# eduardburlacu/DiTSep

Hardware: AMD Instinct MI355X
Metric: separated utterances/sec @ N=30, 2-spk 4 s mixtures (higher is better)
Workload: dtype fp16 (fp16 MFMA operands, fp32 accumulate)

## Files before the change

ditsep_amd/csrc/common.h:

```cpp
#pragma once
#include <hip/hip_runtime.h>
#include <stdint.h>

typedef unsigned short op16_t;
typedef __attribute__((ext_vector_type(8))) unsigned short op16x8;
typedef __attribute__((ext_vector_type(4))) unsigned short op16x4;
typedef __attribute__((ext_vector_type(8))) __bf16 bf16x8;
typedef __attribute__((ext_vector_type(8))) _Float16 f16x8;
typedef __attribute__((ext_vector_type(4))) float f32x4;

#define DSN_WAVE 64

#define DSN_PL(planes, f16) ((planes) | ((f16) << 4))
#define PL_COUNT(pl) ((pl)&3)
#define PL_F16(pl) ((pl) >> 4)

enum { DSN_ACT_NONE = 0, DSN_ACT_ELU = 1, DSN_ACT_SNAKE = 2, DSN_ACT_SILU = 3 };
enum { DSN_F32_NONE = 0, DSN_F32_TANH = 1 };

__device__ __forceinline__ float dsn_elu(float v) { return v > 0.f ? v : expm1f(v); }
__device__ __forceinline__ float dsn_silu(float v) { return v / (1.f + __expf(-v)); }
__device__ __forceinline__ float dsn_snake(float v, float alpha, float inv_beta) {
  float s = __sinf(v * alpha);
  return v + inv_beta * s * s;
}

#define DSN_F16_MAX 65504.f
__device__ __forceinline__ float dsn_sat16(float v) {
  const float c = __builtin_amdgcn_fmed3f(v, -DSN_F16_MAX, DSN_F16_MAX);
  return v != v ? v : c;
}
__device__ __forceinline__ op16_t to_op16(float v, int f16) {
  return f16 ? __builtin_bit_cast(unsigned short, (_Float16)dsn_sat16(v)) : __builtin_bit_cast(unsigned short, (__bf16)v);
}
__device__ __forceinline__ float from_op16(op16_t u, int f16) {
  return f16 ? (float)__builtin_bit_cast(_Float16, u) : (float)__builtin_bit_cast(__bf16, u);
// ... 131 lines not shown
```

ditsep_amd/csrc/engine.hip:

```cpp
#include <math.h>
#include <stdarg.h>
#include <stdio.h>
#include <stdlib.h>
#include <string.h>

#include <algorithm>
#include <map>
#include <numeric>
#include <set>
#include <stdexcept>
#include <string>
#include <vector>

#include "../../include/ditsep_hip.h"
#include "igemm.h"
#include "kernels.h"

namespace {

struct Err : std::runtime_error {
  int code;
  Err(int c, const std::string& m) : std::runtime_error(m), code(c) {}
};

// ... 1664 lines not shown
    if (ctx->fin_err_host && *ctx->fin_err_host) {
      *ctx->fin_err_host = 0;
      fail(DSN_EHIP, "a GroupNorm hand-off wait of an earlier call gave up (the workgroups of one conv were not resident "
                     "together): that call's results are invalid; DSN_NO_GN_FIN=1 selects the separate GroupNorm pass");
    }
    f();
    return DSN_OK;
  } catch (const Err& e) {
    ctx->err = e.what();
    return e.code;
  } catch (const std::exception& e) {
    ctx->err = e.what();
    return DSN_EINVAL;
  }
}
}

extern "C" {

dsn_ctx* dsn_create(const dsn_config* cfg) {
  try {
    if (!cfg) fail(DSN_EINVAL, "null config");
    if (cfg->precision < DSN_PREC_BF16 || cfg->precision > DSN_PREC_FP8)
      fail(DSN_EINVAL, "precision must be one of DSN_PREC_{BF16,BF16X3,FP16,FP16X3,FP8}");
    if (cfg->vae_n_blocks < 0 || cfg->vae_n_blocks > DSN_MAX_VAE_BLOCKS) fail(DSN_EINVAL, "bad vae_n_blocks");
    if (cfg->n_src < 1 || cfg->latent_dim % 32 != 0) fail(DSN_EINVAL, "bad n_src / latent_dim");
    if (cfg->score_kind == DSN_SCORE_DIT &&
        (cfg->dit_heads <= 0 || cfg->dit_embed_dim <= 0 || cfg->dit_embed_dim % cfg->dit_heads != 0 ||
         cfg->dit_embed_dim / cfg->dit_heads != 64))
      fail(DSN_EINVAL, "DiT: only 64-wide attention heads are implemented (embed_dim %d / %d heads = %d)",
           cfg->dit_embed_dim, cfg->dit_heads, cfg->dit_heads > 0 ? cfg->dit_embed_dim / cfg->dit_heads : 0);
// ... 1448 lines not shown
        d.X = t->x;
        d.b7 = t->bias;
        d.b1 = t->bias2;
        d.out_f32 = t->out_f32;
        d.out_planes = oplanes;
        d.out_ps = t->out_ps;
        d.act_mid = t->act;
        d.mid_a = t->act_a;
        d.mid_b = t->act_b;
        d.act_out = t->act_out;
        d.out_a = t->out_act_a;
        d.out_b = t->out_act_b;
        d.S = t->B;
        d.L = t->L;
        d.dil = t->dil;
        const hipError_t e = ru_fused_launch(d, PL, st);
        if (e != hipSuccess)
          fail(DSN_EHIP, "test_kernel ru_fused: refused or failed: %s (S=%d L=%d dil=%d act %d / %d)", hipGetErrorString(e),
               t->B, t->L, t->dil, t->act, t->act_out);
        break;
      }
      case DSN_TK_PC_PRIOR:
      case DSN_TK_PC_CORRECTOR:
      case DSN_TK_PC_PREDICTOR:
      case DSN_TK_MIX_PRIOR:
      case DSN_TK_MIX_CORRECTOR:
      case DSN_TK_MIX_PREDICTOR:
      case DSN_TK_SB_UPDATE:
      case DSN_TK_REPEAT_SOURCES: {
        static const char* const names[] = {"pc_prior", "pc_corrector", "", "pc_predictor", "", "mix_prior",
                                            "mix_corrector", "mix_predictor", "sb_update", "repeat_sources"};
// ... 60 lines not shown
        if (t->B < 1 || t->D < 1 || t->T < 1)
          fail(DSN_EINVAL, "test_kernel vae_sample: B, D, T must be positive (B=%d D=%d T=%d)", t->B, t->D, t->T);
        if (!t->x || !t->z || !t->out_f32) fail(DSN_EINVAL, "test_kernel vae_sample: x (encoder output), z or out_f32 missing");
        launch_vae_sample(t->x, t->z, t->out_f32, t->B, t->D, t->T, st);
        break;
      }
      case DSN_TK_RANDN:
      case DSN_TK_RAND_UNIFORM: {
        const char* nm = t->kind == DSN_TK_RANDN ? "randn" : "rand_uniform";
        if (t->count < 1) fail(DSN_EINVAL, "test_kernel %s: count %ld must be positive", nm, (long)t->count);
        if (!t->out_f32) fail(DSN_EINVAL, "test_kernel %s: out_f32 missing", nm);
        if (t->kind == DSN_TK_RANDN) launch_randn(t->out_f32, (long)t->count, t->seed, t->offset, st);
        else launch_rand_uniform(t->out_f32, (long)t->count, t->seed, t->offset, t->lo, t->hi, st);
        break;
      }
      default:
        fail(DSN_EINVAL, "test_kernel: unknown kind %d", t->kind);
    }
    HIPCHK(hipGetLastError());
  });
}

int dsn_bench_igemm(dsn_ctx* ctx, int B, int Lin, int Cin, int N, int taps, int tap_dil, int in_pad, int ksplit,
                    int variant, int iters, double* ms_out) {
  return guarded(ctx, [&] {
    const int P = ctx->P, PL = ctx->PL;
    const long an = (long)B * Lin * Cin, wn = (long)N * taps * Cin, on = (long)B * Lin * N;
    float* af = ctx->wsbuf<float>("b_af", an);
    float* wf = ctx->wsbuf<float>("b_wf", wn);
    op16_t* ap = ctx->wsbuf<op16_t>("b_a", an * P);
// ... 50 lines not shown
```

ditsep_amd/csrc/igemm.hip:

```cpp
#include "igemm.h"

#ifndef DSN_SETPRIO
#define DSN_SETPRIO 0
#endif

namespace {

constexpr int BM = 128, BN = 128, BK = 32;
constexpr int TILE_ELEMS = 128 * BK;

__device__ __forceinline__ int swz(int row, int chunk) { return chunk ^ ((-(row >> 2)) & 3); }

enum { EPI_STATS = 1, EPI_LNFOLD = 2, EPI_FP8OUT = 4 };
enum { LEAN_NO_DIT = 1, LEAN_NO_NCSN = 2, LEAN_SEEDED = 4 };

template <int NT, int MT>
__device__ __forceinline__ void seed_acc(const GemmDesc& d, f32x4 (&acc)[NT][MT], int mw0, int m_end, int nw0, int lane) {
  const int nq = (lane >> 4) * 4;
#pragma unroll
  for (int tm = 0; tm < MT; ++tm) {
    const int m = mw0 + tm * 16 + (lane & 15);
    const bool mok = m < m_end;
    const int b = mok ? m / d.rows_per_b : 0;
    const int j = mok ? m - b * d.rows_per_b : 0;
// ... 160 lines not shown
      dsn_touch(bg[tp]);
    }
#pragma unroll
    for (int tm = 0; tm < MT; ++tm) {
      const int m = mw0 + tm * 16 + (lane & 15);
      if (m >= m_end) continue;
      const float mu = ln_rows[2 * (m - ln_m0)], rs = ln_rows[2 * (m - ln_m0) + 1];
      f32x4 h[2];
      float amax = 0.f;
#pragma unroll
      for (int tp = 0; tp < 2; ++tp) {
        const f32x4 val = (acc[2 * tp][tm] - cv[tp] * mu) * rs + bv[tp];
        const f32x4 gate = (acc[2 * tp + 1][tm] - cg[tp] * mu) * rs + bg[tp];
#pragma unroll
        for (int r = 0; r < 4; ++r) {
          h[tp][r] = val[r] * dsn_silu(gate[r]);
          amax = fmaxf(amax, fabsf(h[tp][r]));
        }
      }
      amax = fmaxf(amax, __shfl_xor(amax, 16, 64));
      amax = fmaxf(amax, __shfl_xor(amax, 32, 64));
      const int k = dsn_mx_exp(amax);
      const float inv = dsn_pow2(-k);
      const long orow = (long)m * (d.N >> 1);
#pragma unroll
      for (int tp = 0; tp < 2; ++tp)
        *reinterpret_cast<unsigned*>(d.out_fp8 + orow + (nw0 >> 1) + tp * 16 + nq) = dsn_fp8x4(h[tp] * inv);
      if ((lane >> 4) == 0) d.out_fp8_scale[(long)m * (d.N >> 6) + (nw0 >> 6)] = (unsigned char)(k + 127);
    }
    return;
  }
// ... 9 lines not shown
      dsn_touch(cv);
      dsn_touch(cg);
      dsn_touch(bv);
      dsn_touch(bg);
#pragma unroll
      for (int tm = 0; tm < MT; ++tm) {
        const int m = mw0 + tm * 16 + (lane & 15);
        if (m >= m_end) continue;
        const float mu = ln_rows[2 * (m - ln_m0)], rs = ln_rows[2 * (m - ln_m0) + 1];
        const f32x4 val = (acc[2 * tp][tm] - cv * mu) * rs + bv;
        const f32x4 gate = (acc[2 * tp + 1][tm] - cg * mu) * rs + bg;
        op16x4 hi, lo;
#pragma unroll
        for (int r = 0; r < 4; ++r) {
          op16_t h, l;
          dsn_split(val[r] * dsn_silu(gate[r]), h, l, F16);
          hi[r] = h;
          lo[r] = l;
        }
        const long off = (long)m * (d.N >> 1) + (np >> 1) + nq;
        *reinterpret_cast<op16x4*>(d.out_planes + off) = hi;
        if (P == 2) *reinterpret_cast<op16x4*>(d.out_planes + d.out_ps + off) = lo;
      }
    }
    return;
  }
  constexpr bool ROPE_FIRST = MT <= 2;
  if (ROPE_FIRST && !f_swiglu && f_rope) {
    const int section = nw0 / d.qkv_D;
    if (section < 2 && (nw0 & 63) == 0) {
#pragma unroll
// ... 119 lines not shown
      }
    } else if ((EPI & EPI_FP8OUT) && d.out_fp8) {
      static_assert(!(EPI & EPI_FP8OUT) || NT == 4, "fp8 SwiGLU epilogue expects 64 packed columns per wave");
      f32x4 h[2];
      float amax = 0.f;
#pragma unroll
      for (int tp = 0; tp < 2; ++tp) {
        const int np = nw0 + tp * 32;
        f32x4 val = acc[2 * tp][tm], gate = acc[2 * tp + 1][tm];
        if (d.bias && np < d.N) {
          val += *reinterpret_cast<const f32x4*>(d.bias + np + nq);
          gate += *reinterpret_cast<const f32x4*>(d.bias + np + 16 + nq);
        }
#pragma unroll
        for (int r = 0; r < 4; ++r) {
          h[tp][r] = val[r] * dsn_silu(gate[r]);
          amax = fmaxf(amax, fabsf(h[tp][r]));
        }
      }
      amax = fmaxf(amax, __shfl_xor(amax, 16, 64));
      amax = fmaxf(amax, __shfl_xor(amax, 32, 64));
      const int k = dsn_mx_exp(amax);
      const float inv = dsn_pow2(-k);
      if (nw0 < d.N) {
        const long orow = (long)m * (d.N >> 1);
#pragma unroll
        for (int tp = 0; tp < 2; ++tp)
          *reinterpret_cast<unsigned*>(d.out_fp8 + orow + (nw0 >> 1) + tp * 16 + nq) = dsn_fp8x4(h[tp] * inv);
        if ((lane >> 4) == 0) d.out_fp8_scale[(long)m * (d.N >> 6) + (nw0 >> 6)] = (unsigned char)(k + 127);
      }
    } else {
#pragma unroll
      for (int tp = 0; tp < NT / 2; ++tp) {
        const int np = nw0 + tp * 32;
        if (np >= d.N) continue;
        const int feat = (np >> 1) + nq;
        const long off = row_abs + feat;
        f32x4 val = acc[2 * tp][tm], gate = acc[2 * tp + 1][tm];
        if (d.bias) {
          val += *reinterpret_cast<const f32x4*>(d.bias + np + nq);
          gate += *reinterpret_cast<const f32x4*>(d.bias + np + 16 + nq);
        }
        op16x4 hi, lo;
#pragma unroll
        for (int r = 0; r < 4; ++r) {
          op16_t h, l;
          dsn_split(val[r] * dsn_silu(gate[r]), h, l, F16);
          hi[r] = h;
          lo[r] = l;
        }
        *reinterpret_cast<op16x4*>(d.out_planes + off) = hi;
        if (P == 2) *reinterpret_cast<op16x4*>(d.out_planes + d.out_ps + off) = lo;
      }
    }
  }
  if (f_gn && mw0 < m_end) {
    const int b = mw0 / d.rows_per_b;
    const int slice = (mw0 - b * d.rows_per_b) >> 6;
    const int S = d.rows_per_b >> 6;
#pragma unroll
    for (int tn = 0; tn < NT; ++tn) {
      float cnt = (float)(MT * 4);
// ... 1486 lines not shown
```

ditsep_amd/csrc/ru_fused.hip:

```cpp
#include "igemm.h"
#include "kernels.h"
#include <cstdlib>
#include <functional>

namespace {

constexpr int C = 128;
constexpr int TL = 128;
constexpr int KT = 32;
constexpr int WTILE = 128 * KT;
constexpr int NSTW = 3;

__device__ __forceinline__ int swz32(int row, int chunk) { return chunk ^ ((-(row >> 2)) & 3); }

template <int P, int F16>
__global__ __launch_bounds__(256, 2) void ru_fused_kernel(const RuDesc d, const op16_t* __restrict__ zero_page) {
  extern __shared__ __attribute__((aligned(16))) op16_t lds[];
  const int halo = 3 * d.dil;
  const int hrows = (TL + 2 * halo + 3) & ~3;
  constexpr int AH_ROWS = TL + 54 + 2;
  constexpr int AH_PLANE = AH_ROWS * C;
  op16_t* ah = lds;
  op16_t* ring = lds + P * AH_PLANE;
  constexpr int RING_STAGE = P * WTILE;

  const int tid = threadIdx.x, lane = tid & 63;
  const int wave = __builtin_amdgcn_readfirstlane(tid >> 6);
  const int wm = wave >> 1, wn = wave & 1;
  const int tiles_per_seq = (d.L + TL - 1) / TL;
  const int s = blockIdx.x / tiles_per_seq;
// ... 73 lines not shown
#pragma unroll
      for (int tm = 0; tm < 4; ++tm) {
        if (P == 2) {
          acc[tn][tm] = mfma16<F16>(fw[P - 1][tn], fa[0][tm], acc[tn][tm]);
          acc[tn][tm] = mfma16<F16>(fw[0][tn], fa[P - 1][tm], acc[tn][tm]);
        }
        acc[tn][tm] = mfma16<F16>(fw[0][tn], fa[0][tm], acc[tn][tm]);
      }
  }
  asm volatile("s_waitcnt lgkmcnt(0)" ::: "memory");
  __builtin_amdgcn_s_barrier();

  issue_w(d.W1, d.w1_ps, C, 0, 0);
  issue_w(d.W1, d.w1_ps, C, KT, 1);
  const int nq = (lane >> 4) * 4;
#pragma unroll
  for (int tm = 0; tm < 4; ++tm) {
    const int m = wm * 64 + tm * 16 + (lane & 15);
#pragma unroll
    for (int tn = 0; tn < 4; ++tn) {
      const int n = wn * 64 + tn * 16 + nq;
      f32x4 v = acc[tn][tm] + *reinterpret_cast<const f32x4*>(d.b7 + n);
      op16x4 hi, lo;
#pragma unroll
      for (int r = 0; r < 4; ++r) {
        float a = v[r];
        if (d.act_mid == DSN_ACT_ELU) a = dsn_elu(a);
        else if (d.act_mid == DSN_ACT_SNAKE) a = dsn_snake(a, d.mid_a[n + r], d.mid_b[n + r]);
        op16_t h, l;
        dsn_split(a, h, l, F16);
        hi[r] = h;
        lo[r] = l;
      }
      const int off = m * C + (((n >> 3) + 2 * m) & 15) * 8 + (n & 7);
      *reinterpret_cast<op16x4*>(ah + off) = hi;
      if (P == 2) *reinterpret_cast<op16x4*>(ah + AH_PLANE + off) = lo;
      acc[tn][tm] = f32x4{0.f, 0.f, 0.f, 0.f};
    }
  }

  constexpr int NKT1 = C / KT;
  for (int i = 0; i < NKT1; ++i) {
    if (i + 1 < NKT1)
// ... 20 lines not shown
          acc[tn][tm] = mfma16<F16>(fw[P - 1][tn], fa[0][tm], acc[tn][tm]);
          acc[tn][tm] = mfma16<F16>(fw[0][tn], fa[P - 1][tm], acc[tn][tm]);
        }
        acc[tn][tm] = mfma16<F16>(fw[0][tn], fa[0][tm], acc[tn][tm]);
      }
  }

  f32x4 res[4], nres[4];
  auto load_res = [&](int tm, f32x4 (&r)[4]) {
    const int l = l0 + wm * 64 + tm * 16 + (lane & 15);
    const long rowoff = seq_off + (long)min(l, d.L - 1) * C;
#pragma unroll
    for (int tn = 0; tn < 4; ++tn) r[tn] = *reinterpret_cast<const f32x4*>(d.X + rowoff + wn * 64 + tn * 16 + nq);
  };
  load_res(0, res);
#pragma unroll
  for (int tm = 0; tm < 4; ++tm) {
    if (tm + 1 < 4) load_res(tm + 1, nres);
    const int l = l0 + wm * 64 + tm * 16 + (lane & 15);
    const long rowoff = seq_off + (long)l * C;
#pragma unroll
    for (int tn = 0; tn < 4; ++tn) {
      if (l >= d.L) continue;
      const int n = wn * 64 + tn * 16 + nq;
      f32x4 v = acc[tn][tm] + *reinterpret_cast<const f32x4*>(d.b1 + n) + res[tn];
      if (d.out_f32) *reinterpret_cast<f32x4*>(d.out_f32 + rowoff + n) = v;
      if (d.out_planes) {
        op16x4 hi, lo;
#pragma unroll
        for (int r = 0; r < 4; ++r) {
          float a = v[r];
          if (d.act_out == DSN_ACT_ELU) a = dsn_elu(a);
          else if (d.act_out == DSN_ACT_SNAKE) a = dsn_snake(a, d.out_a[n + r], d.out_b[n + r]);
          op16_t h, lw;
          dsn_split(a, h, lw, F16);
          hi[r] = h;
          lo[r] = lw;
        }
        *reinterpret_cast<op16x4*>(d.out_planes + rowoff + n) = hi;
        if (P == 2) *reinterpret_cast<op16x4*>(d.out_planes + d.out_ps + rowoff + n) = lo;
      }
    }
#pragma unroll
    for (int tn = 0; tn < 4; ++tn) res[tn] = nres[tn];
  }
}

constexpr int TL2 = 256;
constexpr int ACH_ROWS = 384;
constexpr int ACH_STAGE = ACH_ROWS * KT;
constexpr int RING2_OFF = 2 * ACH_STAGE;
constexpr int H_ELEMS = TL2 * C;
constexpr int LDS2_ELEMS = H_ELEMS + 2 * WTILE;

template <int F16>
__global__ __launch_bounds__(512, 4) void ru_fused2_kernel(const RuDesc d, const op16_t* __restrict__ zero_page) {
  extern __shared__ __attribute__((aligned(16))) op16_t lds[];
  const int halo = 3 * d.dil;
  const int tid = threadIdx.x, lane = tid & 63;
  const int wave = __builtin_amdgcn_readfirstlane(tid >> 6);
  const int wm = wave >> 1, wn = wave & 1;
  const int tiles_per_seq = (d.L + TL2 - 1) / TL2;
  const int s = blockIdx.x / tiles_per_seq;
  const int l0 = (blockIdx.x - s * tiles_per_seq) * TL2;
  const long seq_off = (long)s * d.L * C;
  const int nrows = TL2 + 2 * halo;

  const op16_t* a_src[3];
#pragma unroll
  for (int j = 0; j < 3; ++j) {
    const int q = (wave * 3 + j) * 64 + lane;
    const int row = q >> 2, c = (q & 3) ^ ((row >> 1) & 3);
    const int l = l0 - halo + row;
    a_src[j] = (row < nrows && l >= 0 && l < d.L) ? d.A + seq_off + (long)l * C + c * 8 : nullptr;
  }
  auto issue_a = [&](int kc) {
#pragma unroll
    for (int j = 0; j < 3; ++j) {
      const op16_t* g = a_src[j] ? a_src[j] + kc * KT : zero_page + (lane & 3) * 8;
      __builtin_amdgcn_global_load_lds((const __attribute__((address_space(1))) void*)g,
                                       (__attribute__((address_space(3))) void*)(lds + (kc & 1) * ACH_STAGE +
                                                                                  (wave * 3 + j) * 64 * 8),
                                       16, 0, 0);
    }
  };
  const int rsub = lane >> 2, cpos = lane & 3;
  const int wrow = wave * 16 + rsub;
  const int wcol = (cpos ^ swz32(wrow, 0)) * 8;
  auto issue_w = [&](const op16_t* W, int ktot, int koff, op16_t* stage) {
    __builtin_amdgcn_global_load_lds(
        (const __attribute__((address_space(1))) void*)(W + (long)wrow * ktot + koff + wcol),
        (__attribute__((address_space(3))) void*)(stage + wave * 16 * KT), 16, 0, 0);
  };

  f32x4 acc[4][4];
#pragma unroll
  for (int a = 0; a < 4; ++a)
#pragma unroll
    for (int b = 0; b < 4; ++b) acc[a][b] = f32x4{0.f, 0.f, 0.f, 0.f};
  const int frow = lane & 15, fchunk = lane >> 4;
  const int w_frag = (wn * 64 + frow) * KT + swz32(frow, fchunk) * 8;
  op16_t* ring = lds + RING2_OFF;

  issue_a(0);
  issue_w(d.W7, 7 * C, 0, ring);
  issue_w(d.W7, 7 * C, C, ring + WTILE);
  int st = 0;
  for (int kc = 0; kc < 4; ++kc) {
    const op16_t* ach = lds + (kc & 1) * ACH_STAGE;
#pragma unroll
    for (int tap = 0; tap < 7; ++tap) {
      if (kc == 3 && tap == 6)
        asm volatile("s_waitcnt vmcnt(0) lgkmcnt(0)" ::: "memory");
      else if ((tap == 1 || tap == 2) && kc < 3)
        asm volatile("s_waitcnt vmcnt(4) lgkmcnt(0)" ::: "memory");
      else
        asm volatile("s_waitcnt vmcnt(1) lgkmcnt(0)" ::: "memory");
      __builtin_amdgcn_s_barrier();
      {
        int t2 = tap + 2, k2 = kc;
        if (t2 >= 7) { t2 -= 7; ++k2; }
        int s2 = st + 2;
        if (s2 >= NSTW) s2 -= NSTW;
        if (k2 < 4) issue_w(d.W7, 7 * C, t2 * C + k2 * KT, ring + s2 * WTILE);
        if (tap == 0 && kc < 3) issue_a(kc + 1);
      }
      const op16_t* wb = ring + st * WTILE;
      op16x8 fa[4], fw[4];
#pragma unroll
      for (int k = 0; k < 4; ++k) {
        const int row = wm * 64 + k * 16 + frow + tap * d.dil;
        fa[k] = *reinterpret_cast<const op16x8*>(ach + row * KT + ((fchunk ^ ((row >> 1) & 3)) * 8));
        fw[k] = *reinterpret_cast<const op16x8*>(wb + w_frag + k * 16 * KT);
      }
#pragma unroll
      for (int tn = 0; tn < 4; ++tn)
#pragma unroll
        for (int tm = 0; tm < 4; ++tm) acc[tn][tm] = mfma16<F16>(fw[tn], fa[tm], acc[tn][tm]);
      if (++st == NSTW) st = 0;
    }
  }
  asm volatile("s_waitcnt lgkmcnt(0)" ::: "memory");
  __builtin_amdgcn_s_barrier();

  op16_t* ring1 = lds + H_ELEMS;
  issue_w(d.W1, C, 0, ring1);
  issue_w(d.W1, C, KT, ring1 + WTILE);
  const int nq = (lane >> 4) * 4;
#pragma unroll
  for (int tm = 0; tm < 4; ++tm) {
    const int m = wm * 64 + tm * 16 + (lane & 15);
#pragma unroll
    for (int tn = 0; tn < 4; ++tn) {
      const int n = wn * 64 + tn * 16 + nq;
      f32x4 v = acc[tn][tm] + *reinterpret_cast<const f32x4*>(d.b7 + n);
      op16x4 hi;
#pragma unroll
      for (int r = 0; r < 4; ++r) {
        float a = v[r];
        if (d.act_mid == DSN_ACT_ELU) a = dsn_elu(a);
        else if (d.act_mid == DSN_ACT_SNAKE) a = dsn_snake(a, d.mid_a[n + r], d.mid_b[n + r]);
        op16_t h, l;
        dsn_split(a, h, l, F16);
        hi[r] = h;
      }
      *reinterpret_cast<op16x4*>(lds + m * C + (((n >> 3) + 2 * m) & 15) * 8 + (n & 7)) = hi;
      const int ls = l0 + wm * 64 + tm * 16 + (lane & 15);
      acc[tn][tm] = *reinterpret_cast<const f32x4*>(d.b1 + n) +
                    *reinterpret_cast<const f32x4*>(d.X + seq_off + (long)min(ls, d.L - 1) * C + n);
    }
  }

#pragma unroll
  for (int i = 0; i < 4; ++i) {
    if (i == 0)
      asm volatile("s_waitcnt vmcnt(1) lgkmcnt(0)" ::: "memory");
    else
      asm volatile("s_waitcnt vmcnt(0) lgkmcnt(0)" ::: "memory");
    __builtin_amdgcn_s_barrier();
    if (i >= 1 && i + 1 < 4) issue_w(d.W1, C, (i + 1) * KT, ring1 + ((i + 1) & 1) * WTILE);
    const op16_t* wb = ring1 + (i & 1) * WTILE;
    op16x8 fa[4], fw[4];
#pragma unroll
    for (int k = 0; k < 4; ++k) {
      const int row = wm * 64 + k * 16 + frow;
      fa[k] = *reinterpret_cast<const op16x8*>(lds + row * C + ((i * 4 + fchunk + 2 * row) & 15) * 8);
      fw[k] = *reinterpret_cast<const op16x8*>(wb + w_frag + k * 16 * KT);
    }
#pragma unroll
    for (int tn = 0; tn < 4; ++tn)
#pragma unroll
      for (int tm = 0; tm < 4; ++tm) acc[tn][tm] = mfma16<F16>(fw[tn], fa[tm], acc[tn][tm]);
  }

#pragma unroll
  for (int tm = 0; tm < 4; ++tm) {
    const int l = l0 + wm * 64 + tm * 16 + (lane & 15);
    const long rowoff = seq_off + (long)l * C;
#pragma unroll
    for (int tn = 0; tn < 4; ++tn) {
      if (l >= d.L) continue;
      const int n = wn * 64 + tn * 16 + nq;
      const f32x4 v = acc[tn][tm];
      if (d.out_f32) *reinterpret_cast<f32x4*>(d.out_f32 + rowoff + n) = v;
      if (d.out_planes) {
        op16x4 hi;
#pragma unroll
        for (int r = 0; r < 4; ++r) {
          float a = v[r];
          if (d.act_out == DSN_ACT_ELU) a = dsn_elu(a);
          else if (d.act_out == DSN_ACT_SNAKE) a = dsn_snake(a, d.out_a[n + r], d.out_b[n + r]);
          op16_t h, lw;
          dsn_split(a, h, lw, F16);
          hi[r] = h;
        }
        *reinterpret_cast<op16x4*>(d.out_planes + rowoff + n) = hi;
      }
    }
  }
}

const op16_t* ru_zero_page() {
  static op16_t* zp[64] = {};
  op16_t*& z = zp[dsn_current_device()];
  if (!z) {
    if (hipMalloc((void**)&z, 4096) != hipSuccess) return nullptr;
    (void)hipMemset(z, 0, 4096);
  }
  return z;
}

template <int P, int F16>
hipError_t launch_t(const RuDesc& d, hipStream_t st) {
  const op16_t* zp = ru_zero_page();
  if (!zp) return hipErrorOutOfMemory;
  const size_t smem = ((size_t)P * (TL + 56) * C + (size_t)NSTW * P * WTILE) * sizeof(op16_t);
  static std::atomic<unsigned long long> attr{0};
  if (dsn_first_use_on_device(attr)) {
    (void)hipFuncSetAttribute(reinterpret_cast<const void*>(ru_fused_kernel<P, F16>),
                              hipFuncAttributeMaxDynamicSharedMemorySize, 160 * 1024);
  }
  const int grid = d.S * ((d.L + TL - 1) / TL);
  hipLaunchKernelGGL((ru_fused_kernel<P, F16>), dim3(grid), dim3(256), smem, st, d, zp);
  return hipGetLastError();
}

}

template <int F16>
hipError_t launch2_t(const RuDesc& d, hipStream_t st) {
  const op16_t* zp = ru_zero_page();
  if (!zp) return hipErrorOutOfMemory;
  const size_t smem = (size_t)LDS2_ELEMS * sizeof(op16_t);
  static std::atomic<unsigned long long> attr{0};
  if (dsn_first_use_on_device(attr)) {
    (void)hipFuncSetAttribute(reinterpret_cast<const void*>(ru_fused2_kernel<F16>),
                              hipFuncAttributeMaxDynamicSharedMemorySize, 160 * 1024);
  }
  const int grid = d.S * ((d.L + TL2 - 1) / TL2);
  hipLaunchKernelGGL((ru_fused2_kernel<F16>), dim3(grid), dim3(512), smem, st, d, zp);
  return hipGetLastError();
}

static bool ru_act_ok(int kind, const float* a, const float* b) {
  if (kind == DSN_ACT_SNAKE) return a && b;
  return kind == DSN_ACT_NONE || kind == DSN_ACT_ELU;
}

hipError_t ru_fused_launch(const RuDesc& d, int pl, hipStream_t st) {
  if (d.dil < 1 || d.dil > 9 || d.S <= 0 || d.L <= 0) return hipErrorInvalidValue;
  if (!d.A || !d.X || !d.W7 || !d.W1 || !d.b7 || !d.b1 || (!d.out_f32 && !d.out_planes)) return hipErrorInvalidValue;
  if (!ru_act_ok(d.act_mid, d.mid_a, d.mid_b)) return hipErrorInvalidValue;
  if (d.out_planes && !ru_act_ok(d.act_out, d.out_a, d.out_b)) return hipErrorInvalidValue;
  const int P = PL_COUNT(pl), f16 = PL_F16(pl);
  if (d.out_planes) {
    const long n = (long)d.S * d.L * C;
    for (int p = 0; p < P; ++p)
      for (int q = 0; q < P; ++q) {
        const op16_t *a = d.A + p * d.a_ps, *o = d.out_planes + q * d.out_ps;
        if (std::less<const op16_t*>()(a, o + n) && std::less<const op16_t*>()(o, a + n)) return hipErrorInvalidValue;
      }
  }
  const bool v1 = getenv("DSN_RU_V1") != nullptr;
  if (P == 1 && !v1) return f16 ? launch2_t<1>(d, st) : launch2_t<0>(d, st);
  if (P == 1) return f16 ? launch_t<1, 1>(d, st) : launch_t<1, 0>(d, st);
  return f16 ? launch_t<2, 1>(d, st) : launch_t<2, 0>(d, st);
}
```

ditsep_amd/native.py:

```python
from __future__ import annotations

import ctypes as C
import math
import os
import warnings
from typing import Mapping, Optional

import torch

_HERE = os.path.dirname(os.path.abspath(__file__))
LIB_PATH = os.environ.get("DSN_LIB", os.path.join(_HERE, "libditsep_hip.so"))

PREC_BF16 = 1
PREC_BF16X3 = 2
PREC_FP16 = 3
PREC_FP16X3 = 4
PREC_FP8 = 5
SCORE_NONE, SCORE_DIT, SCORE_NCSNPP = 0, 1, 2
MAX_VAE_BLOCKS = 8

EXPORTS = [
    "dsn_create", "dsn_destroy", "dsn_last_error", "dsn_load_tensor", "dsn_finalize_weights", "dsn_finalize_weights_ex",
    "dsn_score", "dsn_score_ragged", "dsn_pc_sample_ragged", "dsn_ouve_schedule", "dsn_pc_sample", "dsn_pc_sample_sched", "dsn_pc_sample_ex", "dsn_pc_sample_mix", "dsn_sb_sample", "dsn_decode",
    "dsn_encode", "dsn_decode_chunked", "dsn_encode_chunked",
# ... 102 lines not shown
        ("resid", C.c_void_p), ("resid_bstride", C.c_int64), ("resid_row_elems", C.c_int), ("resid_off", C.c_int),
        ("out_scale", C.c_float), ("f32_op", C.c_int), ("act", C.c_int), ("act_a", C.c_void_p), ("act_b", C.c_void_p),
        ("act_mod", C.c_int), ("swiglu", C.c_int), ("gn_stats", C.c_void_p), ("gn_stats2", C.c_void_p),
        ("gn_nq2", C.c_int), ("gn_qoff2", C.c_int),
        ("sc_a", C.c_void_p), ("sc_a_numel", C.c_int64), ("sc_w", C.c_void_p), ("sc_bias", C.c_void_p),
        ("sc_Cin", C.c_int), ("sc_row_elems", C.c_int),
        ("out_f32", C.c_void_p), ("out_planes", C.c_void_p), ("out_ps", C.c_int64),
        ("slabs", C.c_void_p), ("slab_stride", C.c_int64),
    ]


TEST_KERNEL_KINDS = {"attention": 1, "qkv_attention": 2, "residual_norm": 3, "gn_stats": 4, "gn_apply": 5, "fir2d": 6,
                     "conv_out1": 7, "conv_in1": 8, "ru_fused": 9,
                     "pc_prior": 10, "pc_corrector": 11, "pc_item_norms": 12, "pc_predictor": 13, "sigma_mix": 14,
                     "mix_prior": 15, "mix_corrector": 16, "mix_predictor": 17, "sb_update": 18, "repeat_sources": 19,
                     "vae_sample": 20, "randn": 21, "rand_uniform": 22}


class DsnTestKernel(C.Structure):
    _fields_ = [
        ("kind", C.c_int), ("B", C.c_int), ("S", C.c_int), ("H", C.c_int), ("dh", C.c_int), ("D", C.c_int),
        ("ipp", C.c_int), ("rows", C.c_int), ("nslab", C.c_int), ("do_norm", C.c_int), ("eps", C.c_float),
        ("slab_stride", C.c_int64),
        ("C", C.c_int), ("HW", C.c_int), ("rstride", C.c_int), ("img_h", C.c_int), ("img_w", C.c_int), ("up", C.c_int),
        ("silu", C.c_int), ("bstride", C.c_int64),
        ("L", C.c_int), ("ktaps", C.c_int), ("apply_tanh", C.c_int), ("act", C.c_int),
        ("dil", C.c_int), ("act_out", C.c_int),
        ("a", C.c_void_p), ("a_numel", C.c_int64), ("w", C.c_void_p), ("w_numel", C.c_int64), ("w2", C.c_void_p),
        ("w2_numel", C.c_int64), ("x", C.c_void_p),
        ("slabs", C.c_void_p), ("bias", C.c_void_p), ("bias2", C.c_void_p), ("gamma", C.c_void_p), ("beta", C.c_void_p),
        ("stats", C.c_void_p), ("add", C.c_void_p), ("act_a", C.c_void_p), ("act_b", C.c_void_p),
        ("out_act_a", C.c_void_p), ("out_act_b", C.c_void_p), ("rope_cos", C.c_void_p), ("rope_sin", C.c_void_p),
        ("out_f32", C.c_void_p), ("out_planes", C.c_void_p), ("out_ps", C.c_int64), ("out_fp8", C.c_void_p),
        ("out_fp8_scale", C.c_void_p),
        ("n", C.c_int), ("T", C.c_int), ("avg_len", C.c_int), ("em", C.c_int), ("mean_full", C.c_int),
        ("third_is_y", C.c_int),
        ("stdT", C.c_float), ("step", C.c_float), ("gain", C.c_float), ("snr", C.c_float), ("theta", C.c_float),
        ("dt", C.c_float), ("G", C.c_float), ("g", C.c_float), ("s1", C.c_float), ("s2", C.c_float), ("lam", C.c_float),
        ("sqdt", C.c_float), ("w_prev", C.c_float), ("w_est", C.c_float), ("w3", C.c_float), ("lo", C.c_float),
        ("hi", C.c_float),
        ("seed", C.c_uint64), ("offset", C.c_uint64), ("count", C.c_int64),
        ("y", C.c_void_p), ("score", C.c_void_p), ("z", C.c_void_p), ("smix", C.c_void_p), ("norms", C.c_void_p),
        ("xmean", C.c_void_p),
        ("lens", C.c_void_p),
    ]


def latent_frames_of(L: int, hop: int) -> int:
    return int(L) // int(hop) + 1


def ragged_extended_length(L: int, hop: int) -> int:
    return latent_frames_of(L, hop) * int(hop) - 1


def frame_groups(frames) -> dict:
    groups: dict = {}
    for i, f in enumerate(frames):
        groups.setdefault(int(f), []).append(i)
# ... 649 lines not shown
                assert v.dtype == (torch.int16 if k == "out_planes" else torch.float32), k
                keep.append(v)
                setattr(t, k, v.data_ptr())
                if k == "sc_a":
                    t.sc_a_numel = v.numel()
                if k == "out_planes" and "out_ps" not in kw:
                    t.out_ps = v.shape[-1] if v.dim() > 1 else v.numel()
            elif v is not None:
                setattr(t, k, v)
        self._check(self.lib.dsn_test_gemm(self.ctx, C.byref(t), self._stream()), f"dsn_test_gemm({kernel})")

    def test_kernel(self, kind, **kw):
        t = DsnTestKernel()
        t.kind = TEST_KERNEL_KINDS[kind]
        keep = []
        dtypes = {"out_planes": torch.int16, "out_fp8": torch.uint8, "out_fp8_scale": torch.uint8, "lens": torch.int32}
        for k, v in kw.items():
            if isinstance(v, torch.Tensor):
                assert v.is_cuda and v.dtype == dtypes.get(k, torch.float32), k
                assert v.is_contiguous() or k == "x", k
                keep.append(v)
                setattr(t, k, v.data_ptr())
                if k in ("a", "w", "w2"):
                    setattr(t, k + "_numel", v.numel())
                if k == "out_planes" and "out_ps" not in kw:
                    t.out_ps = v.shape[-1] if v.dim() > 1 else v.numel()
            elif v is not None:
                setattr(t, k, v)
        self._check(self.lib.dsn_test_kernel(self.ctx, C.byref(t), self._stream()), f"dsn_test_kernel({kind})")

    def decode_planes(self, raw):
# ... 5 lines not shown
```

include/ditsep_hip.h:

```cpp
#ifndef DITSEP_HIP_H
#define DITSEP_HIP_H

#include <stdint.h>

#ifdef __cplusplus
extern "C" {
#endif

#define DSN_OK 0
#define DSN_EINVAL (-1)
#define DSN_EHIP (-2)
#define DSN_ESTATE (-3)
#define DSN_ENOMEM (-4)
#define DSN_ESOLVER (-5)

#define DSN_PREC_BF16 1
#define DSN_PREC_BF16X3 2
#define DSN_PREC_FP16 3
#define DSN_PREC_FP16X3 4
#define DSN_PREC_FP8 5

#define DSN_SCORE_NONE 0
#define DSN_SCORE_DIT 1
#define DSN_SCORE_NCSNPP 2
// ... 210 lines not shown
  const float* sc_bias;
  int sc_Cin, sc_row_elems;
  float* out_f32;
  int16_t* out_planes;
  int64_t out_ps;
  float* slabs;
  int64_t slab_stride;
} DsnTestGemm;
int dsn_test_gemm(dsn_ctx* ctx, const DsnTestGemm* t, void* stream);

enum { DSN_TK_ATTENTION = 1, DSN_TK_QKV_ATTENTION = 2, DSN_TK_RESIDUAL_NORM = 3, DSN_TK_GN_STATS = 4,
       DSN_TK_GN_APPLY = 5, DSN_TK_FIR2D = 6, DSN_TK_CONV_OUT1 = 7, DSN_TK_CONV_IN1 = 8, DSN_TK_RU_FUSED = 9,
       DSN_TK_PC_PRIOR = 10, DSN_TK_PC_CORRECTOR = 11, DSN_TK_PC_ITEM_NORMS = 12, DSN_TK_PC_PREDICTOR = 13,
       DSN_TK_SIGMA_MIX = 14, DSN_TK_MIX_PRIOR = 15, DSN_TK_MIX_CORRECTOR = 16, DSN_TK_MIX_PREDICTOR = 17,
       DSN_TK_SB_UPDATE = 18, DSN_TK_REPEAT_SOURCES = 19, DSN_TK_VAE_SAMPLE = 20, DSN_TK_RANDN = 21,
       DSN_TK_RAND_UNIFORM = 22 };
typedef struct DsnTestKernel {
  int kind;
  int B, S, H, dh, D, ipp;
  int rows, nslab, do_norm;
  float eps;
  int64_t slab_stride;
  int C, HW, rstride, img_h, img_w, up, silu;
  int64_t bstride;
  int L, ktaps, apply_tanh, act;
  int dil, act_out;
  const float* a;
  int64_t a_numel;
  const float* w;
  int64_t w_numel;
  const float* w2;
// ... 16 lines not shown
  int16_t* out_planes;
  int64_t out_ps;
  uint8_t* out_fp8;
  uint8_t* out_fp8_scale;
  int n, T, avg_len, em, mean_full, third_is_y;
  float stdT, step, gain, snr, theta, dt, G, g, s1, s2, lam, sqdt, w_prev, w_est, w3, lo, hi;
  uint64_t seed, offset;
  int64_t count;
  const float* y;
  const float* score;
  const float* z;
  const float* smix;
  const float* norms;
  float* xmean;
  const int32_t* lens;
} DsnTestKernel;
int dsn_test_kernel(dsn_ctx* ctx, const DsnTestKernel* t, void* stream);

int dsn_debug_read(dsn_ctx* ctx, const char* name, float* host, int64_t count);
int dsn_bench_igemm(dsn_ctx* ctx, int B, int Lin, int Cin, int N, int taps, int tap_dil, int in_pad, int ksplit,
                    int variant, int iters, double* ms_out);

#ifdef __cplusplus
}
#endif
#endif
```

Measured before the change: 291.9.

## Specialize residual-unit kernels on activation kind and use branch-free ELU/SiLU

Templates the fused residual-unit kernels on the mid and output activation kinds, so ELU and Snake paths are resolved at compile time and Snake alpha/beta are preloaded as vectors instead of per-element loads. It adds a select-based expm1 for non-positive inputs that avoids divergent expm1f calls, and a SiLU that uses a hardware reciprocal in the gated GEMM epilogues. ru_fused2 also gets register-pressure tweaks: offsets in place of pointers, scalar-pinned bases and dilation, and a recomputed lane id. A bit-exact sweep test kernel is added to check the custom expm1 against expm1f, while the rcp-based SiLU may differ slightly in rounding.

New measurement: 293.9, median of 6. No clear change (+0.7%).

```diff
diff --git a/ditsep_amd/csrc/common.h b/ditsep_amd/csrc/common.h
--- a/ditsep_amd/csrc/common.h
+++ b/ditsep_amd/csrc/common.h
@@ -18,8 +18,28 @@
 enum { DSN_ACT_NONE = 0, DSN_ACT_ELU = 1, DSN_ACT_SNAKE = 2, DSN_ACT_SILU = 3 };
 enum { DSN_F32_NONE = 0, DSN_F32_TANH = 1 };
 
+__device__ __forceinline__ float dsn_expm1_nonpos(float v) {
+  const float fn = __builtin_rintf(v * 0x1.715476p+0f);
+  float t = __builtin_fmaf(fn, -0x1.62e430p-1f, v);
+  t = __builtin_fmaf(fn, 0x1.05c610p-29f, t);
+  float p = __builtin_fmaf(0x1.a26762p-13f, t, 0x1.6d2e00p-10f);
+  p = __builtin_fmaf(t, p, 0x1.110ff2p-7f);
+  p = __builtin_fmaf(t, p, 0x1.555502p-5f);
+  p = __builtin_fmaf(t, p, 0x1.555556p-3f);
+  p = __builtin_fmaf(t, p, 0.5f);
+  p = t * p;
+  const float e = __builtin_amdgcn_ldexpf(1.f, (int)fn);
+  const float q = __builtin_fmaf(t, p, t);
+  const float r = __builtin_fmaf(e, q, e - 1.f);
+  return v < -17.f ? -1.f : r;
+}
 __device__ __forceinline__ float dsn_elu(float v) { return v > 0.f ? v : expm1f(v); }
+__device__ __forceinline__ float dsn_elu_sel(float v) {
+  const float e = dsn_expm1_nonpos(v);
+  return v > 0.f ? v : e;
+}
 __device__ __forceinline__ float dsn_silu(float v) { return v / (1.f + __expf(-v)); }
+__device__ __forceinline__ float dsn_silu_rcp(float v) { return v * __builtin_amdgcn_rcpf(1.f + __expf(-v)); }
 __device__ __forceinline__ float dsn_snake(float v, float alpha, float inv_beta) {
   float s = __sinf(v * alpha);
   return v + inv_beta * s * s;
diff --git a/ditsep_amd/csrc/engine.hip b/ditsep_amd/csrc/engine.hip
--- a/ditsep_amd/csrc/engine.hip
+++ b/ditsep_amd/csrc/engine.hip
@@ -1702,7 +1702,31 @@
     return DSN_EINVAL;
   }
 }
-}
+
+__global__ void expm1_sweep_kernel(unsigned first, long count, unsigned* __restrict__ res) {
+  unsigned bad = 0, lowest = 0xffffffffu;
+  for (long i = (long)blockIdx.x * blockDim.x + threadIdx.x; i < count; i += (long)gridDim.x * blockDim.x) {
+    const unsigned bits = first + (unsigned)i;
+    const float v = __builtin_bit_cast(float, bits);
+    const float want = expm1f(v), got = dsn_expm1_nonpos(v);
+    const bool same = __builtin_bit_cast(unsigned, want) == __builtin_bit_cast(unsigned, got) || (want != want && got != got);
+    if (!same) {
+      ++bad;
+      lowest = min(lowest, bits);
+    }
+  }
+  if (bad) {
+    atomicAdd(res, bad);
+    atomicMin(res + 1, lowest);
+  }
+}
+__global__ void elu_values_kernel(const float* __restrict__ x, float* __restrict__ out, long count) {
+  const long i = (long)blockIdx.x * blockDim.x + threadIdx.x;
+  if (i < count) out[i] = dsn_elu_sel(x[i]);
+}
+}
+
+hipError_t ru_fused_launch_ex(const RuDesc& d, int pl, bool generic, hipStream_t stream);
 
 extern "C" {
 
@@ -3181,7 +3205,7 @@
         d.S = t->B;
         d.L = t->L;
         d.dil = t->dil;
-        const hipError_t e = ru_fused_launch(d, PL, st);
+        const hipError_t e = ru_fused_launch_ex(d, PL, t->ru_generic != 0, st);
         if (e != hipSuccess)
           fail(DSN_EHIP, "test_kernel ru_fused: refused or failed: %s (S=%d L=%d dil=%d act %d / %d)", hipGetErrorString(e),
                t->B, t->L, t->dil, t->act, t->act_out);
@@ -3272,6 +3296,20 @@
         else launch_rand_uniform(t->out_f32, (long)t->count, t->seed, t->offset, t->lo, t->hi, st);
         break;
       }
+      case DSN_TK_ELU_EXACT: {
+        if (t->count < 1) fail(DSN_EINVAL, "test_kernel elu_exact: count %ld must be positive", (long)t->count);
+        if (t->x) {
+          if (!t->out_f32) fail(DSN_EINVAL, "test_kernel elu_exact: out_f32 missing");
+          hipLaunchKernelGGL(elu_values_kernel, dim3(cdiv(t->count, 256)), dim3(256), 0, st, t->x, t->out_f32, (long)t->count);
+        } else {
+          if (!t->out_u32) fail(DSN_EINVAL, "test_kernel elu_exact: out_u32 (mismatches, first pattern) missing");
+          if (t->offset + (uint64_t)t->count > (1ull << 32))
+            fail(DSN_EINVAL, "test_kernel elu_exact: patterns offset .. offset + count - 1 must fit 32 bits");
+          const int grid = (int)std::min<long>(cdiv(t->count, 256), 1 << 16);
+          hipLaunchKernelGGL(expm1_sweep_kernel, dim3(grid), dim3(256), 0, st, (unsigned)t->offset, (long)t->count, t->out_u32);
+        }
+        break;
+      }
       default:
         fail(DSN_EINVAL, "test_kernel: unknown kind %d", t->kind);
     }
diff --git a/ditsep_amd/csrc/igemm.hip b/ditsep_amd/csrc/igemm.hip
--- a/ditsep_amd/csrc/igemm.hip
+++ b/ditsep_amd/csrc/igemm.hip
@@ -198,7 +198,7 @@
         const f32x4 gate = (acc[2 * tp + 1][tm] - cg[tp] * mu) * rs + bg[tp];
 #pragma unroll
         for (int r = 0; r < 4; ++r) {
-          h[tp][r] = val[r] * dsn_silu(gate[r]);
+          h[tp][r] = val[r] * dsn_silu_rcp(gate[r]);
           amax = fmaxf(amax, fabsf(h[tp][r]));
         }
       }
@@ -238,7 +238,7 @@
 #pragma unroll
         for (int r = 0; r < 4; ++r) {
           op16_t h, l;
-          dsn_split(val[r] * dsn_silu(gate[r]), h, l, F16);
+          dsn_split(val[r] * dsn_silu_rcp(gate[r]), h, l, F16);
           hi[r] = h;
           lo[r] = l;
         }
@@ -388,7 +388,7 @@
         }
 #pragma unroll
         for (int r = 0; r < 4; ++r) {
-          h[tp][r] = val[r] * dsn_silu(gate[r]);
+          h[tp][r] = val[r] * dsn_silu_rcp(gate[r]);
           amax = fmaxf(amax, fabsf(h[tp][r]));
         }
       }
@@ -419,7 +419,7 @@
 #pragma unroll
         for (int r = 0; r < 4; ++r) {
           op16_t h, l;
-          dsn_split(val[r] * dsn_silu(gate[r]), h, l, F16);
+          dsn_split(val[r] * dsn_silu_rcp(gate[r]), h, l, F16);
           hi[r] = h;
           lo[r] = l;
         }
diff --git a/ditsep_amd/csrc/ru_fused.hip b/ditsep_amd/csrc/ru_fused.hip
--- a/ditsep_amd/csrc/ru_fused.hip
+++ b/ditsep_amd/csrc/ru_fused.hip
@@ -13,7 +13,37 @@
 
 __device__ __forceinline__ int swz32(int row, int chunk) { return chunk ^ ((-(row >> 2)) & 3); }
 
-template <int P, int F16>
+__device__ __forceinline__ int fresh_lane() {
+  int l = __builtin_amdgcn_mbcnt_hi(~0u, __builtin_amdgcn_mbcnt_lo(~0u, 0));
+  asm volatile("" : "+v"(l));
+  return l;
+}
+
+constexpr int ACT_RT = -1;
+template <int K>
+struct RuAct {
+  f32x4 al[4], ib[4];
+  __device__ __forceinline__ void load(const float* a, const float* b, int n0) {
+    if constexpr (K == DSN_ACT_SNAKE) {
+#pragma unroll
+      for (int tn = 0; tn < 4; ++tn) {
+        al[tn] = *reinterpret_cast<const f32x4*>(a + n0 + tn * 16);
+        ib[tn] = *reinterpret_cast<const f32x4*>(b + n0 + tn * 16);
+      }
+    }
+  }
+  __device__ __forceinline__ float operator()(float v, int kind, const float* a, const float* b, int tn, int n, int r) const {
+    if constexpr (K == DSN_ACT_ELU) return dsn_elu_sel(v);
+    if constexpr (K == DSN_ACT_SNAKE) return dsn_snake(v, al[tn][r], ib[tn][r]);
+    if constexpr (K == ACT_RT) {
+      if (kind == DSN_ACT_ELU) return dsn_elu_sel(v);
+      if (kind == DSN_ACT_SNAKE) return dsn_snake(v, a[n + r], b[n + r]);
+    }
+    return v;
+  }
+};
+
+template <int P, int F16, int AM, int AO>
 __global__ __launch_bounds__(256, 2) void ru_fused_kernel(const RuDesc d, const op16_t* __restrict__ zero_page) {
   extern __shared__ __attribute__((aligned(16))) op16_t lds[];
   const int halo = 3 * d.dil;
@@ -117,6 +147,8 @@
   issue_w(d.W1, d.w1_ps, C, 0, 0);
   issue_w(d.W1, d.w1_ps, C, KT, 1);
   const int nq = (lane >> 4) * 4;
+  RuAct<AM> act_mid;
+  act_mid.load(d.mid_a, d.mid_b, wn * 64 + nq);
 #pragma unroll
   for (int tm = 0; tm < 4; ++tm) {
     const int m = wm * 64 + tm * 16 + (lane & 15);
@@ -128,8 +160,7 @@
 #pragma unroll
       for (int r = 0; r < 4; ++r) {
         float a = v[r];
-        if (d.act_mid == DSN_ACT_ELU) a = dsn_elu(a);
-        else if (d.act_mid == DSN_ACT_SNAKE) a = dsn_snake(a, d.mid_a[n + r], d.mid_b[n + r]);
+        a = act_mid(a, d.act_mid, d.mid_a, d.mid_b, tn, n, r);
         op16_t h, l;
         dsn_split(a, h, l, F16);
         hi[r] = h;
@@ -180,6 +211,8 @@
     for (int tn = 0; tn < 4; ++tn) r[tn] = *reinterpret_cast<const f32x4*>(d.X + rowoff + wn * 64 + tn * 16 + nq);
   };
   load_res(0, res);
+  RuAct<AO> act_out;
+  act_out.load(d.out_a, d.out_b, wn * 64 + nq);
 #pragma unroll
   for (int tm = 0; tm < 4; ++tm) {
     if (tm + 1 < 4) load_res(tm + 1, nres);
@@ -196,8 +229,7 @@
 #pragma unroll
         for (int r = 0; r < 4; ++r) {
           float a = v[r];
-          if (d.act_out == DSN_ACT_ELU) a = dsn_elu(a);
-          else if (d.act_out == DSN_ACT_SNAKE) a = dsn_snake(a, d.out_a[n + r], d.out_b[n + r]);
+          a = act_out(a, d.act_out, d.out_a, d.out_b, tn, n, r);
           op16_t h, lw;
           dsn_split(a, h, lw, F16);
           hi[r] = h;
@@ -219,7 +251,7 @@
 constexpr int H_ELEMS = TL2 * C;
 constexpr int LDS2_ELEMS = H_ELEMS + 2 * WTILE;
 
-template <int F16>
+template <int F16, int AM, int AO>
 __global__ __launch_bounds__(512, 4) void ru_fused2_kernel(const RuDesc d, const op16_t* __restrict__ zero_page) {
   extern __shared__ __attribute__((aligned(16))) op16_t lds[];
   const int halo = 3 * d.dil;
@@ -232,18 +264,20 @@
   const long seq_off = (long)s * d.L * C;
   const int nrows = TL2 + 2 * halo;
 
-  const op16_t* a_src[3];
+  int a_src[3];
 #pragma unroll
   for (int j = 0; j < 3; ++j) {
     const int q = (wave * 3 + j) * 64 + lane;
     const int row = q >> 2, c = (q & 3) ^ ((row >> 1) & 3);
     const int l = l0 - halo + row;
-    a_src[j] = (row < nrows && l >= 0 && l < d.L) ? d.A + seq_off + (long)l * C + c * 8 : nullptr;
+    a_src[j] = (row < nrows && l >= 0 && l < d.L) ? l * C + c * 8 : -1;
   }
   auto issue_a = [&](int kc) {
+    const op16_t* Ab = d.A + seq_off;
+    asm volatile("" : "+s"(Ab));
 #pragma unroll
     for (int j = 0; j < 3; ++j) {
-      const op16_t* g = a_src[j] ? a_src[j] + kc * KT : zero_page + (lane & 3) * 8;
+      const op16_t* g = a_src[j] >= 0 ? Ab + a_src[j] + kc * KT : zero_page + (lane & 3) * 8;
       __builtin_amdgcn_global_load_lds((const __attribute__((address_space(1))) void*)g,
                                        (__attribute__((address_space(3))) void*)(lds + (kc & 1) * ACH_STAGE +
                                                                                   (wave * 3 + j) * 64 * 8),
@@ -274,6 +308,8 @@
   int st = 0;
   for (int kc = 0; kc < 4; ++kc) {
     const op16_t* ach = lds + (kc & 1) * ACH_STAGE;
+    int dil = d.dil;
+    asm volatile("" : "+s"(dil));
 #pragma unroll
     for (int tap = 0; tap < 7; ++tap) {
       if (kc == 3 && tap == 6)
@@ -295,7 +331,7 @@
       op16x8 fa[4], fw[4];
 #pragma unroll
       for (int k = 0; k < 4; ++k) {
-        const int row = wm * 64 + k * 16 + frow + tap * d.dil;
+        const int row = wm * 64 + k * 16 + frow + tap * dil;
         fa[k] = *reinterpret_cast<const op16x8*>(ach + row * KT + ((fchunk ^ ((row >> 1) & 3)) * 8));
         fw[k] = *reinterpret_cast<const op16x8*>(wb + w_frag + k * 16 * KT);
       }
@@ -310,28 +346,37 @@
   __builtin_amdgcn_s_barrier();
 
   op16_t* ring1 = lds + H_ELEMS;
-  issue_w(d.W1, C, 0, ring1);
-  issue_w(d.W1, C, KT, ring1 + WTILE);
-  const int nq = (lane >> 4) * 4;
-#pragma unroll
-  for (int tm = 0; tm < 4; ++tm) {
-    const int m = wm * 64 + tm * 16 + (lane & 15);
-#pragma unroll
-    for (int tn = 0; tn < 4; ++tn) {
-      const int n = wn * 64 + tn * 16 + nq;
+  const int lane_e = fresh_lane();
+  const int nq = (lane_e >> 4) * 4, lrow = lane_e & 15;
+  const int w1_off = (wave * 16 + (lane_e >> 2)) * C + ((lane_e & 3) ^ swz32(wave * 16 + (lane_e >> 2), 0)) * 8;
+  const op16_t* W1 = d.W1;
+  asm volatile("" : "+s"(W1));
+  auto issue_w1 = [&](int koff, op16_t* stage) {
+    __builtin_amdgcn_global_load_lds((const __attribute__((address_space(1))) void*)(W1 + w1_off + koff),
+                                     (__attribute__((address_space(3))) void*)(stage + wave * 16 * KT), 16, 0, 0);
+  };
+  issue_w1(0, ring1);
+  issue_w1(KT, ring1 + WTILE);
+  RuAct<AM> act_mid;
+  act_mid.load(d.mid_a, d.mid_b, wn * 64 + nq);
+#pragma unroll
+  for (int tn = 0; tn < 4; ++tn) {
+    const int n = wn * 64 + tn * 16 + nq;
+#pragma unroll
+    for (int tm = 0; tm < 4; ++tm) {
+      const int m = wm * 64 + tm * 16 + lrow;
       f32x4 v = acc[tn][tm] + *reinterpret_cast<const f32x4*>(d.b7 + n);
       op16x4 hi;
 #pragma unroll
       for (int r = 0; r < 4; ++r) {
         float a = v[r];
-        if (d.act_mid == DSN_ACT_ELU) a = dsn_elu(a);
-        else if (d.act_mid == DSN_ACT_SNAKE) a = dsn_snake(a, d.mid_a[n + r], d.mid_b[n + r]);
+        a = act_mid(a, d.act_mid, d.mid_a, d.mid_b, tn, n, r);
         op16_t h, l;
         dsn_split(a, h, l, F16);
         hi[r] = h;
       }
       *reinterpret_cast<op16x4*>(lds + m * C + (((n >> 3) + 2 * m) & 15) * 8 + (n & 7)) = hi;
-      const int ls = l0 + wm * 64 + tm * 16 + (lane & 15);
+      const int ls = l0 + wm * 64 + tm * 16 + lrow;
       acc[tn][tm] = *reinterpret_cast<const f32x4*>(d.b1 + n) +
                     *reinterpret_cast<const f32x4*>(d.X + seq_off + (long)min(ls, d.L - 1) * C + n);
     }
@@ -344,14 +389,14 @@
     else
       asm volatile("s_waitcnt vmcnt(0) lgkmcnt(0)" ::: "memory");
     __builtin_amdgcn_s_barrier();
-    if (i >= 1 && i + 1 < 4) issue_w(d.W1, C, (i + 1) * KT, ring1 + ((i + 1) & 1) * WTILE);
-    const op16_t* wb = ring1 + (i & 1) * WTILE;
+    if (i >= 1 && i + 1 < 4) issue_w1((i + 1) * KT, ring1 + ((i + 1) & 1) * WTILE);
+    const op16_t* wb = ring1 + (i & 1) * WTILE + (wn * 64 + lrow) * KT + swz32(lrow, lane_e >> 4) * 8;
     op16x8 fa[4], fw[4];
 #pragma unroll
     for (int k = 0; k < 4; ++k) {
-      const int row = wm * 64 + k * 16 + frow;
-      fa[k] = *reinterpret_cast<const op16x8*>(lds + row * C + ((i * 4 + fchunk + 2 * row) & 15) * 8);
-      fw[k] = *reinterpret_cast<const op16x8*>(wb + w_frag + k * 16 * KT);
+      const int row = wm * 64 + k * 16 + lrow;
+      fa[k] = *reinterpret_cast<const op16x8*>(lds + row * C + ((i * 4 + (lane_e >> 4) + 2 * row) & 15) * 8);
+      fw[k] = *reinterpret_cast<const op16x8*>(wb + k * 16 * KT);
     }
 #pragma unroll
     for (int tn = 0; tn < 4; ++tn)
@@ -359,9 +404,12 @@
       for (int tm = 0; tm < 4; ++tm) acc[tn][tm] = mfma16<F16>(fw[tn], fa[tm], acc[tn][tm]);
   }
 
+  RuAct<AO> act_out;
+  act_out.load(d.out_a, d.out_b, wn * 64 + nq);
+  const int orow = fresh_lane() & 15;
 #pragma unroll
   for (int tm = 0; tm < 4; ++tm) {
-    const int l = l0 + wm * 64 + tm * 16 + (lane & 15);
+    const int l = l0 + wm * 64 + tm * 16 + orow;
     const long rowoff = seq_off + (long)l * C;
 #pragma unroll
     for (int tn = 0; tn < 4; ++tn) {
@@ -374,8 +422,7 @@
 #pragma unroll
         for (int r = 0; r < 4; ++r) {
           float a = v[r];
-          if (d.act_out == DSN_ACT_ELU) a = dsn_elu(a);
-          else if (d.act_out == DSN_ACT_SNAKE) a = dsn_snake(a, d.out_a[n + r], d.out_b[n + r]);
+          a = act_out(a, d.act_out, d.out_a, d.out_b, tn, n, r);
           op16_t h, lw;
           dsn_split(a, h, lw, F16);
           hi[r] = h;
@@ -396,36 +443,53 @@
   return z;
 }
 
-template <int P, int F16>
+template <int P, int F16, int AM, int AO>
 hipError_t launch_t(const RuDesc& d, hipStream_t st) {
   const op16_t* zp = ru_zero_page();
   if (!zp) return hipErrorOutOfMemory;
   const size_t smem = ((size_t)P * (TL + 56) * C + (size_t)NSTW * P * WTILE) * sizeof(op16_t);
   static std::atomic<unsigned long long> attr{0};
   if (dsn_first_use_on_device(attr)) {
-    (void)hipFuncSetAttribute(reinterpret_cast<const void*>(ru_fused_kernel<P, F16>),
+    (void)hipFuncSetAttribute(reinterpret_cast<const void*>(ru_fused_kernel<P, F16, AM, AO>),
                               hipFuncAttributeMaxDynamicSharedMemorySize, 160 * 1024);
   }
   const int grid = d.S * ((d.L + TL - 1) / TL);
-  hipLaunchKernelGGL((ru_fused_kernel<P, F16>), dim3(grid), dim3(256), smem, st, d, zp);
+  hipLaunchKernelGGL((ru_fused_kernel<P, F16, AM, AO>), dim3(grid), dim3(256), smem, st, d, zp);
   return hipGetLastError();
 }
 
-}
-
-template <int F16>
+template <int F16, int AM, int AO>
 hipError_t launch2_t(const RuDesc& d, hipStream_t st) {
   const op16_t* zp = ru_zero_page();
   if (!zp) return hipErrorOutOfMemory;
   const size_t smem = (size_t)LDS2_ELEMS * sizeof(op16_t);
   static std::atomic<unsigned long long> attr{0};
   if (dsn_first_use_on_device(attr)) {
-    (void)hipFuncSetAttribute(reinterpret_cast<const void*>(ru_fused2_kernel<F16>),
+    (void)hipFuncSetAttribute(reinterpret_cast<const void*>(ru_fused2_kernel<F16, AM, AO>),
                               hipFuncAttributeMaxDynamicSharedMemorySize, 160 * 1024);
   }
   const int grid = d.S * ((d.L + TL2 - 1) / TL2);
-  hipLaunchKernelGGL((ru_fused2_kernel<F16>), dim3(grid), dim3(512), smem, st, d, zp);
+  hipLaunchKernelGGL((ru_fused2_kernel<F16, AM, AO>), dim3(grid), dim3(512), smem, st, d, zp);
   return hipGetLastError();
+}
+
+template <int V, int AM, int AO>
+hipError_t launch_v(const RuDesc& d, int f16, hipStream_t st) {
+  if constexpr (V == 0) return f16 ? launch2_t<1, AM, AO>(d, st) : launch2_t<0, AM, AO>(d, st);
+  else return f16 ? launch_t<V, 1, AM, AO>(d, st) : launch_t<V, 0, AM, AO>(d, st);
+}
+template <int V>
+hipError_t launch_acts(const RuDesc& d, int f16, bool generic, hipStream_t st) {
+  const int am = d.act_mid, ao = d.out_planes ? d.act_out : DSN_ACT_NONE;
+  if (!generic) {
+    if (am == DSN_ACT_ELU && ao == DSN_ACT_ELU) return launch_v<V, DSN_ACT_ELU, DSN_ACT_ELU>(d, f16, st);
+    if (am == DSN_ACT_ELU && ao == DSN_ACT_NONE) return launch_v<V, DSN_ACT_ELU, DSN_ACT_NONE>(d, f16, st);
+    if (am == DSN_ACT_SNAKE && ao == DSN_ACT_SNAKE) return launch_v<V, DSN_ACT_SNAKE, DSN_ACT_SNAKE>(d, f16, st);
+    if (am == DSN_ACT_SNAKE && ao == DSN_ACT_NONE) return launch_v<V, DSN_ACT_SNAKE, DSN_ACT_NONE>(d, f16, st);
+  }
+  return launch_v<V, ACT_RT, ACT_RT>(d, f16, st);
+}
+
 }
 
 static bool ru_act_ok(int kind, const float* a, const float* b) {
@@ -433,7 +497,7 @@
   return kind == DSN_ACT_NONE || kind == DSN_ACT_ELU;
 }
 
-hipError_t ru_fused_launch(const RuDesc& d, int pl, hipStream_t st) {
+hipError_t ru_fused_launch_ex(const RuDesc& d, int pl, bool generic, hipStream_t st) {
   if (d.dil < 1 || d.dil > 9 || d.S <= 0 || d.L <= 0) return hipErrorInvalidValue;
   if (!d.A || !d.X || !d.W7 || !d.W1 || !d.b7 || !d.b1 || (!d.out_f32 && !d.out_planes)) return hipErrorInvalidValue;
   if (!ru_act_ok(d.act_mid, d.mid_a, d.mid_b)) return hipErrorInvalidValue;
@@ -448,7 +512,9 @@
       }
   }
   const bool v1 = getenv("DSN_RU_V1") != nullptr;
-  if (P == 1 && !v1) return f16 ? launch2_t<1>(d, st) : launch2_t<0>(d, st);
-  if (P == 1) return f16 ? launch_t<1, 1>(d, st) : launch_t<1, 0>(d, st);
-  return f16 ? launch_t<2, 1>(d, st) : launch_t<2, 0>(d, st);
-}
+  if (P == 1 && !v1) return launch_acts<0>(d, f16, generic, st);
+  if (P == 1) return launch_acts<1>(d, f16, generic, st);
+  return launch_acts<2>(d, f16, generic, st);
+}
+
+hipError_t ru_fused_launch(const RuDesc& d, int pl, hipStream_t st) { return ru_fused_launch_ex(d, pl, false, st); }
diff --git a/ditsep_amd/native.py b/ditsep_amd/native.py
--- a/ditsep_amd/native.py
+++ b/ditsep_amd/native.py
@@ -140,7 +140,7 @@
                      "conv_out1": 7, "conv_in1": 8, "ru_fused": 9,
                      "pc_prior": 10, "pc_corrector": 11, "pc_item_norms": 12, "pc_predictor": 13, "sigma_mix": 14,
                      "mix_prior": 15, "mix_corrector": 16, "mix_predictor": 17, "sb_update": 18, "repeat_sources": 19,
-                     "vae_sample": 20, "randn": 21, "rand_uniform": 22}
+                     "vae_sample": 20, "randn": 21, "rand_uniform": 22, "elu_exact": 23}
 
 
 class DsnTestKernel(C.Structure):
@@ -169,6 +169,7 @@
         ("y", C.c_void_p), ("score", C.c_void_p), ("z", C.c_void_p), ("smix", C.c_void_p), ("norms", C.c_void_p),
         ("xmean", C.c_void_p),
         ("lens", C.c_void_p),
+        ("ru_generic", C.c_int), ("out_u32", C.c_void_p),
     ]
 
 
@@ -848,7 +849,8 @@
         t = DsnTestKernel()
         t.kind = TEST_KERNEL_KINDS[kind]
         keep = []
-        dtypes = {"out_planes": torch.int16, "out_fp8": torch.uint8, "out_fp8_scale": torch.uint8, "lens": torch.int32}
+        dtypes = {"out_planes": torch.int16, "out_fp8": torch.uint8, "out_fp8_scale": torch.uint8, "lens": torch.int32,
+                  "out_u32": torch.int32}
         for k, v in kw.items():
             if isinstance(v, torch.Tensor):
                 assert v.is_cuda and v.dtype == dtypes.get(k, torch.float32), k
diff --git a/include/ditsep_hip.h b/include/ditsep_hip.h
--- a/include/ditsep_hip.h
+++ b/include/ditsep_hip.h
@@ -248,7 +248,7 @@
        DSN_TK_PC_PRIOR = 10, DSN_TK_PC_CORRECTOR = 11, DSN_TK_PC_ITEM_NORMS = 12, DSN_TK_PC_PREDICTOR = 13,
        DSN_TK_SIGMA_MIX = 14, DSN_TK_MIX_PRIOR = 15, DSN_TK_MIX_CORRECTOR = 16, DSN_TK_MIX_PREDICTOR = 17,
        DSN_TK_SB_UPDATE = 18, DSN_TK_REPEAT_SOURCES = 19, DSN_TK_VAE_SAMPLE = 20, DSN_TK_RANDN = 21,
-       DSN_TK_RAND_UNIFORM = 22 };
+       DSN_TK_RAND_UNIFORM = 22, DSN_TK_ELU_EXACT = 23 };
 typedef struct DsnTestKernel {
   int kind;
   int B, S, H, dh, D, ipp;
@@ -295,6 +295,8 @@
   const float* norms;
   float* xmean;
   const int32_t* lens;
+  int ru_generic;
+  uint32_t* out_u32;
 } DsnTestKernel;
 int dsn_test_kernel(dsn_ctx* ctx, const DsnTestKernel* t, void* stream);
 
```
